# shaunlebron/blinky

Hardware: AMD Instinct MI355X
Metric: warped Mpixels/s (lensmap apply) (higher is better)
Workload: dtype u8; 1 GPU; 3840x2160 cube/panini f_fov 180, 64 frames/step from a resident ring of 64 distinct globes (1.80 GB, advanced every step), one lensmap; value / ms_per_step = the job with steps alternating between 2 HIP stream(s), value_one_stream = the same on one stream, roofline.kernel_ms_per_launch = the kernel alone under HIP events; 64 frames/step since r5 (r1-r4 ran 16: compare those with value_at_16_frames; ring_globes=64, parallelism=row-stripes x1, streams=2

## Files before the change

blinky_amd/csrc/bk_build_kernels.h:

```cpp

BK_DEV void bk_state_init(BkState &S, const BkBuildParams *P)
{
    S.P = P;
    S.err = 0;
    S.steps = 0;
    S.flag = 0;
    BK_INIT_GLOBALS(S)
}

BK_DEV int bk_ray_to_plate_index(BkState &S, const float *ray)
{
    const BkBuildParams &P = *S.P;
#ifdef BK_HAS_GLOBE_PLATE
    bkv a[3] = {bk_num((double)ray[0]), bk_num((double)ray[1]), bk_num((double)ray[2])};
    bkv r[BK_MAXRET];
    int n = LF_globe_plate(S, a, 3, r);
    if (n < 1 || !bk_isnum(r[n - 1])) return -1;
    double d = r[n - 1].n;
    if (r[n - 1].e != 0.0 && !(bkm_rint(d - r[n - 1].e) == bkm_rint(d + r[n - 1].e))) S.flag = 1;
    if (!(d > -2147483648.0 && d < 2147483647.0)) return -1;
    int plate = (int)bkm_rint(d);
    if (plate < 0 || plate >= P.numplates) return -1;
    return plate;
#else
// ... 112 lines not shown
    if (threadIdx.x < 6) s_disp[threadIdx.x] = 0;
    __syncthreads();
    const int lx = blockIdx.x * blockDim.x + threadIdx.x;
    const int lyl = blockIdx.y;
    const int ly = P.row0 + lyl;
    int err = 0;
    bool flagged = false;
    unsigned int off = 0xFFFFFFFFu;
    unsigned char tint = 255;
    unsigned short sub = 0x8080;
    const size_t o = (size_t)lyl * P.W + lx;
    if (lx < P.W) {
        int plate;
        BkState S;
        bk_state_init(S, &P);
        bk_inverse_entry(P, S, lx, ly, &off, &tint, &plate, P.subtexel ? &sub : nullptr);
        if (plate >= 0 && !S.flag) s_disp[plate] = 1;
        err = S.err;
        P.offsets[o] = off;
        P.tints[o] = tint;
        if (P.subtexel) P.subtexel[o] = sub;
        flagged = S.flag != 0;
        if ((err & BK_ERR_RESULT) && P.first_bad) atomicMax(P.first_bad, (unsigned int)(ly * P.W + (P.W - 1 - lx)) + 1u);
    }
    bk_push_flagged_wave(P, flagged, (unsigned int)o, off, tint, sub);
    __syncthreads();
    bk_publish_flags(s_disp, P.display, err, P.err);
}
#endif
#endif

// ... 404 lines not shown
```

blinky_amd/csrc/bk_emit.cpp:

```cpp
#include "bk_emit.h"

#include <cmath>
#include <cstdio>
#include <map>
#include <set>
#include <sstream>

namespace bk {
using namespace bklua;

namespace {

[[noreturn]] void unsupported(const std::string &chunk, int line, const std::string &what)
{
    throw LuaError(chunk + ":" + std::to_string(line) + ": not supported in a GPU callback: " + what);
}

std::string sanitize(const std::string &s)
{
    std::string o;
    for (char c : s) o += (isalnum((unsigned char)c) ? c : '_');
    return o;
}

// ... 14 lines not shown
};

struct Emitter {
    Interp &I;
    std::map<std::pair<const FuncProto *, std::string>, FnInfo> fns;
    std::vector<std::string> fn_code;
    std::set<std::string> mutable_globals;
    std::map<const Table *, std::pair<std::string, int>> const_tables;
    std::ostringstream table_code;
    int uid = 0;
    struct SinCos { std::string s, c; long epoch; };
    std::map<std::string, SinCos> sincos;
    long epoch = 0;
    struct Pure { std::string name; long epoch; };
    std::map<std::string, Pure> pure;
    std::string last_single, last_single_of;
    static bool is_name(const std::string &v)
    {
        if (v.empty() || (v[0] >= '0' && v[0] <= '9')) return false;
        for (char c : v) if (!(c == '_' || c == '.' || (c >= '0' && c <= '9') || (c >= 'a' && c <= 'z') || (c >= 'A' && c <= 'Z'))) return false;
        return true;
    }
    static bool mentions(const std::string &key, const std::string &var)
    {
        auto word = [](char c) { return c == '_' || c == '.' || (c >= '0' && c <= '9') || (c >= 'a' && c <= 'z') || (c >= 'A' && c <= 'Z'); };
        for (size_t at = key.find(var); at != std::string::npos; at = key.find(var, at + 1)) {
            const bool left = at == 0 || !word(key[at - 1]), right = at + var.size() >= key.size() || !word(key[at + var.size()]);
            if (left && right) return true;
        }
        return false;
// ... 16 lines not shown
    struct Scope {
        const FuncProto *proto = nullptr;
        const Closure *cl = nullptr;
        const Scope *parent = nullptr;
    };
    struct Fn : Scope {
        std::ostringstream out;
        int indent = 1;
        std::map<int, int> array_slots;
        std::map<int, std::string> fn_slots;
        std::set<int> fn_open;
        std::map<int, Value> static_slots;
        std::map<int, std::vector<std::string>> record_slots;
        std::map<int, std::pair<int, int>> matrix_slots;
        std::string lp = "l", ap = "A", rp = "R";
        std::string field_var(int slot, const std::string &name) const { return rp + std::to_string(slot) + "_" + name; }
        bool is_table(int slot) const { return array_slots.count(slot) || record_slots.count(slot) || matrix_slots.count(slot); }
        std::string chunk;
    };
    static const Value *upvalue_of(const Scope *s, int idx, const Scope **owner, int *slot)
    {
        while (!s->cl) {
            const UpvalDesc &d = s->proto->upvals[(size_t)idx];
            if (d.from_parent_local) { *owner = s->parent; *slot = d.index; return nullptr; }
            idx = d.index;
            s = s->parent;
        }
        *owner = nullptr;
        return s->cl->upvals[(size_t)idx].get();
    }
// ... 211 lines not shown
        switch (e.kind) {
        case Expr::Nil: return "bk_nil()";
        case Expr::True: return "bk_bool(true)";
        case Expr::False: return "bk_bool(false)";
        case Expr::Number: return num_literal(e.num);
        case Expr::String: return str_literal(e.str);
        case Expr::Vararg: {
            const std::string np = std::to_string(f.proto->nparams);
            return "(na > " + np + " ? a[" + np + "] : bk_nil())";
        }
        case Expr::Function: unsupported(f.chunk, e.line, "function values / closures");
        case Expr::Table: unsupported(f.chunk, e.line, "table constructors other than 'local t = {a, b, ...}'");
        case Expr::Name: {
            int slot = 0;
            if (Fn *o = local_of(f, e, &slot)) {
                if (o->is_table(slot)) unsupported(f.chunk, e.line, "table '" + e.str + "' used as a value");
                if (o->fn_slots.count(slot)) unsupported(f.chunk, e.line, "function '" + e.str + "' used as a value (a function defined inside a callback can only be called)");
                if (o->static_slots.count(slot))
                    unsupported(f.chunk, e.line, std::string(o->static_slots[slot].t == Value::TABLE ? "table" : "function") + " '" + e.str +
                                                     "' used as a value (it can be " + (o->static_slots[slot].t == Value::TABLE ? "indexed" : "called") + ", and passed on to script functions)");
                return o->lp + std::to_string(slot);
            }
            if (e.var == VarKind::Global && mutable_globals.count(e.str)) return "S.g_" + sanitize(e.str);
            if (e.var == VarKind::Upvalue) {
                const Scope *owner = nullptr;
                if (const std::string *field = cell_field(upvalue_of(&f, e.slot, &owner, &slot))) return "S." + *field;
            }
            {
                Value v;
                static_value(f, e, &v);
// ... 8 lines not shown
                const auto &names = ao->record_slots[aslot];
                for (const std::string &n : names) if (n == e.b->str) return ao->field_var(aslot, n);
                return "bk_nil()";
            }
            if (ao && ao->matrix_slots.count(aslot)) unsupported(f.chunk, e.line, "a row of table '" + e.a->str + "' used as a value");
            if (e.a->kind == Expr::Index) {
                int mslot = 0;
                Fn *mo = local_of(f, *e.a->a, &mslot);
                if (mo && mo->matrix_slots.count(mslot)) {
                    const std::string row = matrix_row(f, *mo, mslot, *e.a->b);
                    const std::string k = emit_expr(f, *e.b), t = tmp();
                    line(f, "bkv " + t + " = bk_aget(S, " + row + ", " + std::to_string(mo->matrix_slots[mslot].second) + ", " + k + ");");
                    return t;
                }
            }
            if (ao && ao->array_slots.count(aslot)) {
                std::string k = emit_expr(f, *e.b), t = tmp();
                line(f, "bkv " + t + " = bk_aget(S, " + ao->ap + std::to_string(aslot) + ", " + std::to_string(ao->array_slots[aslot]) + ", " + k + ");");
                return t;
            }
            Value sv;
            if (static_value(f, e, &sv)) return const_value(f, e, sv, "field '" + e.b->str + "'");
            Value o;
            if (static_value(f, *e.a, &o) && o.t == Value::TABLE) {
                auto ct = const_table(f, e, o.tab_ptr(), e.a->kind == Expr::Name ? e.a->str : "table");
                std::string k = emit_expr(f, *e.b), t = tmp();
                line(f, "bkv " + t + " = bk_aget(S, " + ct.first + ", " + std::to_string(ct.second) + ", " + k + ");");
                return t;
            }
            unsupported(f.chunk, e.line, "indexing this expression");
// ... 144 lines not shown
        }
        return {arr, cnt};
    }

    bool single_valued_call(Fn &f, const Expr &e)
    {
        Value callee;
        if (e.kind != Expr::Call || !e.str.empty() || !static_value(f, *e.a, &callee) || callee.t != Value::BUILTIN) return false;
        const std::string &bn = callee.bi()->name;
        return bn.compare(0, 5, "math.") == 0 && bn != "math.modf" && bn != "math.frexp";
    }

    void emit_call(Fn &f, const Expr &e, std::string *arr, std::string *cnt)
    {
        ad_call.clear();
        Value callee, self_obj;
        const bool method = !e.str.empty();
        if (method) {
            if (!static_value(f, *e.a, &self_obj) || self_obj.t != Value::TABLE)
                unsupported(f.chunk, e.line, "method calls (a:" + e.str + "(..)) on a value that is not a constant table of the script");
            callee = static_field(self_obj, Value::string(e.str));
            if (callee.t != Value::FUNC) unsupported(f.chunk, e.line, "method '" + e.str + "' is not a script function");
        } else {
            int slot = 0;
            Fn *o = local_of(f, *e.a, &slot);
            if (o && o->fn_slots.count(slot)) {
                if (o->fn_open.count(slot)) unsupported(f.chunk, e.line, "recursion ('" + e.a->str + "')");
                *arr = tmp("r");
                *cnt = tmp("n");
                Args a = emit_args(f, e.args);
                auto packed = pack(f, a, 1);
                line(f, "bkv " + *arr + "[BK_MAXRET];");
                line(f, "const int " + *cnt + " = " + o->fn_slots[slot] + "(" + packed.first + ", " + packed.second + ", " + *arr + ");");
                ++epoch;
                return;
            }
        }
        if (!method && !static_value(f, *e.a, &callee)) {
            std::string n = e.a->kind == Expr::Name ? "'" + e.a->str + "'" : "this expression";
            unsupported(f.chunk, e.line, "calling " + n + " (callee must be a script function or builtin known at build time)");
        }
        *arr = tmp("r");
        *cnt = tmp("n");
        if (callee.t == Value::FUNC) {
            std::vector<std::pair<int, Value>> bound;
            std::vector<const Expr *> plain;
            static const Expr nil_expr = [] { Expr x; x.kind = Expr::Nil; return x; }();
            const int shift = method ? 1 : 0;
            if (method) {
// ... 4 lines not shown
            for (size_t i = 0; i < e.args.size(); ++i) {
                Value av;
                const Expr &x = *e.args[i];
                if ((int)i + shift < callee.fn()->proto->nparams && (x.kind == Expr::Name || x.kind == Expr::Index) && static_value(f, x, &av) &&
                    (av.is_function() || av.t == Value::TABLE)) {
                    bound.emplace_back((int)i + shift, av);
                    plain.push_back(&nil_expr);
                } else plain.push_back(&x);
            }
            const FnInfo &fi = ensure_function(callee.fn(), e.line, f.chunk, bound);
            Args a = emit_args(f, plain);
            auto packed = pack(f, a, 1);
            line(f, "bkv " + *arr + "[BK_MAXRET];");
            line(f, "const int " + *cnt + " = " + fi.cname + "(S, " + packed.first + ", " + packed.second + ", " + *arr + ");");
            ++epoch;
            return;
        }
        if (callee.t != Value::BUILTIN) {
            std::string n = e.a->kind == Expr::Name ? e.a->str : "?";
            unsupported(f.chunk, e.line, "attempt to call '" + n + "' (a " + callee.type_name() + " value)");
        }
        const std::string &bn = callee.bi()->name;
        if (bn == "print") {
            line(f, "bkv " + *arr + "[1]; const int " + *cnt + " = 0; (void)" + *arr + ";");
            return;
        }
        Args a = emit_args(f, e.args);
        auto A = [&](size_t i) { return arg_at(a, i); };
        auto single = [&](const std::string &expr) {
            line(f, "bkv " + *arr + "[1] = {" + expr + "}; const int " + *cnt + " = 1;");
// ... 232 lines not shown
        if (ao && ao->record_slots.count(slot)) {
            if (target.b->kind != Expr::String) unsupported(f.chunk, target.line, "indexing record '" + target.a->str + "' with a computed key");
            for (const std::string &n : ao->record_slots[slot]) if (n == target.b->str) { line(f, ao->field_var(slot, n) + " = " + val + ";"); forget(ao->field_var(slot, n)); return; }
            unsupported(f.chunk, target.line, "adding field '" + target.b->str + "' to '" + target.a->str + "' (name it in the constructor)");
        }
        if (target.a->kind == Expr::Index) {
            int mslot = 0;
            Fn *mo = local_of(f, *target.a->a, &mslot);
            if (mo && mo->matrix_slots.count(mslot)) {
                const std::string row = matrix_row(f, *mo, mslot, *target.a->b);
                const std::string k = emit_expr(f, *target.b);
                line(f, "bk_aset(S, " + row + ", " + std::to_string(mo->matrix_slots[mslot].second) + ", " + k + ", " + val + ");");
                return;
            }
        }
        if (ao && ao->array_slots.count(slot)) {
            std::string k = emit_expr(f, *target.b);
            line(f, "bk_aset(S, " + ao->ap + std::to_string(slot) + ", " + std::to_string(ao->array_slots[slot]) + ", " + k + ", " + val + ");");
            return;
        }
        unsupported(f.chunk, target.line, "storing into this table (only tables created by 'local t = {..}' in the same function are writable)");
    }

    static void declare_locals(std::ostream &o, const Fn &f, const std::string &pad)
    {
        const FuncProto *p = f.proto;
        for (int i = 0; i < p->nslots; ++i) {
            if (f.fn_slots.count(i)) continue;
            if (f.record_slots.count(i)) {
                for (const std::string &name : f.record_slots.at(i)) o << pad << "bkv " << f.field_var(i, name) << " = bk_nil();   /* " << p->slot_names[i] << "." << name << " */\n";
            } else if (f.matrix_slots.count(i)) {
                const int cells = f.matrix_slots.at(i).first * f.matrix_slots.at(i).second;
                o << pad << "bkv " << f.ap << i << "[" << cells + 1 << "];   /* " << p->slot_names[i] << " */\n";
                o << pad << "for (int q = 0; q <= " << cells << "; ++q) " << f.ap << i << "[q] = bk_nil();\n";
            } else if (f.array_slots.count(i)) {
                o << pad << "bkv " << f.ap << i << "[" << f.array_slots.at(i) + 1 << "];   /* " << p->slot_names[i] << " */\n";
            } else if (i < p->nparams) {
                o << pad << "bkv " << f.lp << i << " = na > " << i << " ? a[" << i << "] : bk_nil();   /* " << p->slot_names[i] << " */\n";
            } else {
                o << pad << "bkv " << f.lp << i << " = bk_nil();   /* " << p->slot_names[i] << " */\n";
            }
        }
    }

    void emit_local_function(Fn &f, const Stmt &s)
    {
        const FuncProto *p = s.exprs[0]->proto;
        const int slot = s.slots[0];
        if (f.fn_slots.count(slot) || f.is_table(slot)) unsupported(f.chunk, s.line, "re-declaring '" + s.names[0] + "'");
        const std::string id = std::to_string(++uid);
        Fn g;
        g.proto = p;
        g.parent = &f;
        g.chunk = f.chunk;
        g.lp = "n" + id + "_l";
        g.ap = "n" + id + "_A";
        g.rp = "n" + id + "_R";
        g.indent = f.indent + 1;
        const std::string name = "NF" + id + "_" + sanitize(s.names[0]);
        f.fn_slots[slot] = name;
        f.fn_open.insert(slot);
        emit_block(g, p->body);
        f.fn_open.erase(slot);
        line(f, "/* " + f.chunk + ":" + std::to_string(p->line) + "  function " + s.names[0] + " */");
        line(f, "auto " + name + " = [&](const bkv *a, int na, bkv *r) -> int {");
        std::ostringstream decl;
        declare_locals(decl, g, std::string((size_t)(f.indent + 1) * 4, ' '));
        f.out << decl.str();
        line(f, "    (void)a; (void)na; (void)r;");
        f.out << g.out.str();
        line(f, "    return 0;");
        line(f, "};");
    }

    void emit_stmt(Fn &f, const Stmt &s)
    {
        const bool plain = s.kind == Stmt::Local || s.kind == Stmt::Assign;
        if (!plain) ++epoch;
        emit_stmt_body(f, s);
        if (!plain) ++epoch;
    }
    void emit_stmt_body(Fn &f, const Stmt &s)
    {
        switch (s.kind) {
        case Stmt::Local: {
            if (s.slots.size() == 1 && s.exprs.size() == 1 && s.exprs[0]->kind == Expr::Function) { emit_local_function(f, s); return; }
            if (s.slots.size() == 1 && s.exprs.size() == 1 && (s.exprs[0]->kind == Expr::Name || s.exprs[0]->kind == Expr::Index)) {
// ... 41 lines not shown
                return;
            }
            if (s.slots.size() == 1 && s.exprs.size() == 1 && s.exprs[0]->kind == Expr::Table) {
                const Expr &t = *s.exprs[0];
                if (!t.fields.empty()) unsupported(f.chunk, s.line, "table constructors mixing positional and named fields");
                if (!t.args.empty() && t.args.back()->kind == Expr::Call && !single_valued_call(f, *t.args.back()))
                    unsupported(f.chunk, s.line, "call expansion inside a table constructor (write '(f(...))' to keep one value)");
                if (!t.args.empty() && t.args.back()->kind == Expr::Vararg)
                    unsupported(f.chunk, s.line, "'...' at the end of a table constructor (a table of a size only known at run time)");
                std::vector<std::string> vals;
                for (auto &x : t.args) vals.push_back(emit_expr(f, *x));
                int n = (int)vals.size();
                if (f.array_slots.count(s.slots[0]) && f.array_slots[s.slots[0]] != n) unsupported(f.chunk, s.line, "re-declaring a table with a different size");
                if (f.record_slots.count(s.slots[0]) || f.matrix_slots.count(s.slots[0])) unsupported(f.chunk, s.line, "re-declaring a table");
                f.array_slots[s.slots[0]] = n;
                for (int i = 0; i < n; ++i) line(f, f.ap + std::to_string(s.slots[0]) + "[" + std::to_string(i + 1) + "] = " + vals[i] + ";");
                return;
            }
            auto v = emit_values(f, s.exprs, s.slots.size());
            for (size_t i = 0; i < s.slots.size(); ++i) {
                line(f, f.lp + std::to_string(s.slots[i]) + " = " + v[i] + ";");
                forget(f.lp + std::to_string(s.slots[i]));
                if (ad_active && &f == ad_fn && ad_slot.count(s.slots[i])) line(f, ad_slot[s.slots[i]] + " = " + d_of(v[i]) + ";");
            }
            return;
        }
        case Stmt::LocalFunction: emit_local_function(f, s); return;
        case Stmt::Assign: {
            auto v = emit_values(f, s.exprs, s.targets.size());
            for (size_t i = 0; i < s.targets.size(); ++i) store(f, *s.targets[i], v[i]);
            return;
// ... 3 lines not shown
            line(f, "{");
            f.indent++;
            emit_call(f, *s.call, &arr, &cnt);
            line(f, "(void)" + cnt + ";");
            f.indent--;
            line(f, "}");
            return;
        }
        case Stmt::Do:
            line(f, "{");
            f.indent++;
            emit_block(f, s.body);
            f.indent--;
            line(f, "}");
            return;
        case Stmt::While: {
            line(f, "for (;;) {");
            f.indent++;
            line(f, "if (!bk_tick(S)) break;");
            std::string c = emit_expr(f, *s.cond);
            line(f, "if (!bk_truthy(" + c + ")) break;");
            emit_block(f, s.body);
            f.indent--;
            line(f, "}");
            return;
        }
        case Stmt::Repeat: {
            line(f, "for (;;) {");
            f.indent++;
            line(f, "if (!bk_tick(S)) break;");
            emit_block(f, s.body);
            std::string c = emit_expr(f, *s.cond);
            line(f, "if (bk_truthy(" + c + ")) break;");
            f.indent--;
            line(f, "}");
            return;
        }
        case Stmt::If: {
            int opened = 0;
            for (size_t i = 0; i < s.clauses.size(); ++i) {
                const auto &c = s.clauses[i];
                if (!c.first) {
                    emit_block(f, c.second);
                    break;
                }
                std::string cv = emit_expr(f, *c.first);
                line(f, "if (bk_truthy(" + cv + ")) {");
                f.indent++;
                emit_block(f, c.second);
                f.indent--;
// ... 78 lines not shown
            line(f, "const bkv " + gv + " = " + arr + "[" + gi + "];");
            line(f, std::string("if (") + gv + ".t == BK_TNIL) " + (is_ipairs ? "break;" : "continue;"));
            for (size_t i = 0; i < s.slots.size(); ++i)
                line(f, f.lp + std::to_string(s.slots[i]) + " = " + (i == 0 ? "bk_num((double)" + gi + ")" : i == 1 ? gv : std::string("bk_nil()")) + ";");
            emit_block(f, s.body);
            f.indent--;
            line(f, "}");
            return;
        }
        case Stmt::Return: {
            if (s.exprs.size() == 1 && s.exprs[0]->kind == Expr::Call) {
                std::string arr, cnt;
                line(f, "{");
                f.indent++;
                emit_call(f, *s.exprs[0], &arr, &cnt);
                line(f, "for (int q = 0; q < " + cnt + "; ++q) r[q] = " + arr + "[q];");
                line(f, "return " + cnt + ";");
                f.indent--;
                line(f, "}");
                return;
            }
            line(f, "{");
            f.indent++;
            Args a = emit_args(f, s.exprs);
            if (a.fixed.size() > 8) unsupported(f.chunk, s.line, "more than 8 return values");
            if (a.multi && a.fixed.size() > 4) unsupported(f.chunk, s.line, "more than 4 return values in front of a trailing call or `...`");
            for (size_t i = 0; i < a.fixed.size(); ++i) line(f, "r[" + std::to_string(i) + "] = " + a.fixed[i] + ";");
            if (a.multi) {
                line(f, "for (int q = 0; q < " + a.mcnt + " && " + std::to_string(a.fixed.size()) + " + q < BK_MAXRET; ++q) r[" + std::to_string(a.fixed.size()) + " + q] = " + a.marr + "[q];");
                line(f, "return " + std::to_string(a.fixed.size()) + " + " + a.mcnt + ";");
            } else line(f, "return " + std::to_string(a.fixed.size()) + ";");
// ... 22 lines not shown
        if (fi.emitting) unsupported(from_chunk, line_no, "recursion ('" + cl->proto->name + "')");
        fi.proto = cl->proto;
        fi.cl = cl;
        fi.cname = "LF" + std::to_string(++uid) + "_" + sanitize(cl->proto->name);
        fi.emitting = true;

        Fn f;
        f.proto = cl->proto;
        f.cl = cl;
        f.chunk = cl->chunk->name;
        for (auto &b : bound) {
            if (!slot_is_constant(cl->proto, b.first))
                unsupported(from_chunk, line_no, std::string(b.second.t == Value::TABLE ? "a table" : "a function") + " passed as '" + cl->proto->slot_names[(size_t)b.first] + "' of '" + cl->proto->name + "', which assigns or captures that parameter");
            f.static_slots[b.first] = b.second;
        }
        emit_block(f, cl->proto->body);

        std::ostringstream o;
        o << "/* " << f.chunk << ":" << cl->proto->line << "  function " << cl->proto->name << " */\n";
        o << "BK_DEV int " << fi.cname << "(BkState &S, const bkv *a, int na, bkv *r)\n{\n";
        declare_locals(o, f, "    ");
        o << "    (void)a; (void)na; (void)r;\n";
        o << f.out.str();
        o << "    return 0;\n}\n\n";
        fn_code.push_back(o.str());
        fi.emitting = false;
        fi.done = true;
        return fi;
    }
};
// ... 355 lines not shown
```

blinky_amd/csrc/bk_lens.cpp:

```cpp
#include <chrono>
#include <cstring>
#include <future>

#include "bk_emit.h"
#include "bk_lens_priv.h"

using namespace bklua;

namespace bk {

static double need_num(const Values &a, size_t i, const char *fn)
{
    if (i >= a.size() || a[i].t != Value::NUM)
        throw LuaError(std::string("bad argument #") + std::to_string(i + 1) + " to '" + fn + "' (number expected)");
    return a[i].n;
}

LensProgram::LensProgram(bk_ctx *ctx) : interp(math_platform())
{
    interp.print_sink = [this](const std::string &s) { console += s; };
    static const char *alias[] = {"cos", "sin", "tan", "asin", "acos", "atan", "atan2", "sinh", "cosh", "tanh",
                                  "log", "log10", "abs", "sqrt", "exp", "pow"};
    Value math = interp.get_global("math");
    for (const char *a : alias) interp.set_global(a, math.tab()->get(Value::string(a)));
// ... 395 lines not shown
extern "C" int bk_debug_kernel_source(bk_ctx *ctx, char *buf, size_t cap, size_t *needed, int compile)
{
    if (!ctx) return BK_E_INVALID;
    LensProgram *P = ctx->prog;
    if (!P || !P->lens_valid) return ctx->fail(BK_E_STATE, "no valid lens");
    std::string src;
    if (int r = generate_source(ctx, P, &src)) return r;
    if (needed) *needed = src.size() + 1;
    if (buf && cap) snprintf(buf, cap, "%s", src.c_str());
    if (compile) return compile_module(ctx, P, src);
    return BK_OK;
}
#endif

#if BK_DEBUG_API
extern "C" int bk_debug_eval(bk_ctx *ctx, int which, const double *args, int nargs, double *out, int *nout)
{
    if (!ctx || !ctx->prog) return BK_E_INVALID;
    LensProgram *P = ctx->prog;
    const Value &f = which == 0 ? P->lens_inverse : which == 1 ? P->lens_forward : P->globe_plate;
    if (!f.is_function()) return ctx->fail(BK_E_STATE, "callback not defined");
    try {
        Values a;
        for (int i = 0; i < nargs; ++i) a.push_back(Value::number(args[i]));
        P->interp.steps = 0;
        Values r = P->interp.call(f, a);
        *nout = (int)r.size();
        for (size_t i = 0; i < r.size() && i < 8; ++i) out[i] = r[i].t == Value::NUM ? r[i].n : __builtin_nan("");
        if (r.size() == 1 && r[0].t == Value::NIL) *nout = -1;
    } catch (const LuaError &e) {
// ... 27 lines not shown
```

blinky_amd/csrc/bk_modules.cpp:

```cpp
#include <hip/hiprtc.h>

#include <cerrno>
#include <chrono>
#include <cstring>
#include <map>
#include <mutex>
#include <dlfcn.h>
#include <fcntl.h>
#include <spawn.h>
#include <sys/stat.h>
#include <sys/wait.h>
#include <unistd.h>

#include "bk_codecache.h"
#include "bk_emit.h"
#include "bk_modules.h"

using namespace bk;
extern char **environ;

static std::string cache_path(const std::string &source, const std::string &arch)
{
    const std::string dir = cache_dir();
    if (dir.empty()) return std::string();
    Sha256 h;
    h.update(source);
    for (int i = 0; i < bk::kNumEmbeddedHeaders; ++i) h.update(std::string(bk::kEmbeddedHeaders[i].text));
    h.update(arch);
    h.update(std::string(bk_version()));
    h.update(std::string("-O3 -std=c++17 -ffp-contract=off"));
    return dir + "/bk_lens_" + hex128(h) + ".hsaco";
}

static std::mutex g_rtc_mutex;
static std::map<uint64_t, std::shared_ptr<std::vector<char>>> g_rtc_cache;

static uint64_t code_key(const std::string &source, const std::string &arch)
{
    return fnv1a64(arch.data(), arch.size(), fnv1a64(source.data(), source.size()));
}

CodeResult cached_code(const std::string &source, const std::string &arch)
{
    CodeResult r;
    std::lock_guard<std::mutex> lock(g_rtc_mutex);
// ... 15 lines not shown
    CodeResult r = cached_code(source, arch);
    if (r.code) return r;
    std::lock_guard<std::mutex> lock(g_rtc_mutex);
    auto hit = g_rtc_cache.find(code_key(source, arch));
    if (hit != g_rtc_cache.end() && !bk::g_debug.no_memcache) { r.code = hit->second; return r; }
    std::vector<const char *> hnames, htexts;
    for (int i = 0; i < bk::kNumEmbeddedHeaders; ++i) {
        hnames.push_back(bk::kEmbeddedHeaders[i].name);
        htexts.push_back(bk::kEmbeddedHeaders[i].text);
    }
    hiprtcProgram prog;
    if (hiprtcCreateProgram(&prog, source.c_str(), "bk_lens_build.hip", (int)hnames.size(), htexts.data(), hnames.data()) != HIPRTC_SUCCESS) {
        r.rc = BK_E_HIP; r.log = "hiprtcCreateProgram failed";
        return r;
    }
    const char *opts[] = {arch.c_str(), "-O3", "-std=c++17", "-ffp-contract=off"};
    if (hiprtcCompileProgram(prog, 4, opts) != HIPRTC_SUCCESS) {
        size_t n = 0;
        hiprtcGetProgramLogSize(prog, &n);
        std::string log(n, 0);
        if (n) hiprtcGetProgramLog(prog, &log[0]);
        hiprtcDestroyProgram(&prog);
        r.rc = BK_E_HIP; r.log = "hiprtc failed to compile the lens kernels: " + log;
        return r;
    }
    size_t cs = 0;
    hiprtcGetCodeSize(prog, &cs);
    r.code = std::make_shared<std::vector<char>>(cs);
    hiprtcGetCode(prog, r.code->data());
    hiprtcDestroyProgram(&prog);
    store_sealed(cache_path(source, arch), *r.code);
    if (g_rtc_cache.size() >= 64) g_rtc_cache.clear();
// ... 179 lines not shown
```

blinky_amd/ffi.py:

```python
import ctypes as C
import os

import numpy as np

try:
    import torch
except ImportError:
    torch = None

LIB_PATH = os.environ.get("BLINKY_HIP_LIB") or os.path.join(os.path.dirname(os.path.abspath(__file__)), "libblinkyhip.so")
if not os.path.exists(LIB_PATH):
    raise ImportError(
        f"{LIB_PATH} is missing: build it with `python -c 'import __graft_entry__ as g; g.build()'` "
        "(or `make -C blinky_amd/csrc`).  There is no CPU fallback."
    )
lib = C.CDLL(LIB_PATH)

MAX_PLATES = 6
MIP_MAX_LEVELS = 16
NULL_OFFSET = 0xFFFFFFFF
DEVICE_NONE = -2
OK = 0
PENDING = 1
MAP_NONE, MAP_INVERSE, MAP_FORWARD = 0, 1, 2
# ... 83 lines not shown
    "bk_create_palmap": (None, [_vp, _vp]),
    "bk_create_tintmap_rgba": (None, [_vp, _vp]),
    "bk_get_size": (_i, [_vp] + [C.POINTER(_i)] * 5),
    "bk_version": (C.c_char_p, []),
    "bk_set_apply_variant": (_i, [_vp, _i]),
    "bk_set_resident_share": (_i, [_vp, _i, _i, _i]),
    "bk_set_resident_apply": (_i, [_vp, _i]),
    "bk_multi_set_resident_apply": (_i, [_vp, _i]),
    "bk_set_blockmap_tuning": (_i, [_vp, _i]),
    "bk_set_host_compile": (_i, [_i]),
    "bk_host_module_ready": (_i, [_vp, _i]),
    "bk_debug_module_from_cache": (_i, [_vp]),
    "bk_debug_forward_tiles": (_i, [_vp, C.POINTER(_i), C.POINTER(_i)]),
    "bk_debug_set_option": (_i, [C.c_char_p, _i]),
    "bk_debug_build_breakdown": (_i, [_vp, C.POINTER(_d)]),
    "bk_multi_lensmap_valid": (_i, [_vp]),
    "bk_last_build_ms": (_d, [_vp]),
    "bk_globe_pitch": (_i, [_vp]),
    "bk_globe_rows": (_i, [_vp]),
    "bk_globe_texel_offset": (C.c_uint32, [_vp, _i, _i, _i]),
    "bk_download_plate": (_i, [_vp, _i, _i, _vp, _i]),
    "bk_save_plate": (_i, [_vp, _i, _i, _i, _vp, _i]),
    "bk_debug_tile_stats": (_i, [_vp, C.POINTER(_i)]),
    "bk_debug_traffic_model": (_i, [_vp, C.POINTER(C.c_uint64)]),
    "bk_debug_band_balance": (_i, [_vp, C.POINTER(C.c_uint32)]),
    "bk_debug_stream_mix": (_i, [_vp, _sz, _i, _i, C.POINTER(_d)]),
    "bk_debug_fnv1a64": (_i, [_vp, _sz, C.POINTER(C.c_uint64)]),
    "bk_debug_host_build": (_i, [_vp, _i, _vp, _vp, C.POINTER(_i), C.POINTER(_d)]),
    "bk_debug_host_build_subtexel": (_i, [_vp, _i, _vp, _vp, _vp, C.POINTER(_i), C.POINTER(_d)]),
    "bk_debug_resident_latency": (_i, [_vp, _i, _vp, _i, _i, C.POINTER(_d), C.POINTER(_d)]),
# ... 41 lines not shown
    "bk_multi_clear_globe": (_i, [_vp]),
    "bk_multi_resize": (_i, [_vp, _i, _i]),
    "bk_multi_set_frames": (_i, [_vp, _i]),
    "bk_multi_set_zoom": (_i, [_vp, _i, _i]),
    "bk_multi_set_rubixgrid": (_i, [_vp, _i, _d, _d]),
    "bk_multi_upload_plate": (_i, [_vp, _i, _i, _vp, _i]),
    "bk_multi_fill_plate_lcg": (_i, [_vp, _i, _i, C.c_uint32]),
    "bk_multi_synchronize": (_i, [_vp]),
    "bk_multi_build": (_i, [_vp, C.POINTER(_i), C.POINTER(_d)]),
    "bk_multi_apply": (_i, [_vp, _i, _vp, _i, _i, _i, _i, _vp]),
    "bk_multi_apply_stripes": (_i, [_vp, _i, _i, C.POINTER(_vp), _i, _vp]),
    "bk_multi_wait": (_i, [_vp, _i]),
    "bk_multi_gather": (_i, [_vp, C.POINTER(_vp), _i, _i, _vp, _sz, _i]),
    "bk_multi_exchange_rotating": (_i, [_vp, C.POINTER(_vp), _i, C.POINTER(_vp), _sz, _i]),
}
for _name, (_res, _args) in _SIGS.items():
    _fn = getattr(lib, _name)
    _fn.restype, _fn.argtypes = _res, _args

EXPORTS = tuple(_SIGS)


class BlinkyError(RuntimeError):
    pass


def debug_set_option(name, value):
    if lib.bk_debug_set_option(name.encode(), int(value)) != OK:
        raise ValueError(f"bk_debug_set_option: unknown option {name!r}")


# ... 115 lines not shown
    def calc_zoom(self):
        scale = _d()
        self._chk(lib.bk_calc_zoom(self._h, C.byref(scale)))
        return scale.value

    def last_build_fixups(self):
        a, b = _i(), _i()
        self._chk(lib.bk_last_build_fixups(self._h, C.byref(a), C.byref(b)))
        return a.value, b.value

    def build_breakdown(self):
        out = (_d * 6)()
        self._chk(lib.bk_debug_build_breakdown(self._h, out))
        return dict(build_ms=out[0], host_eval_ms=out[1], flagged=int(out[2]), pool_threads=int(out[3]), kernel_wall_ms=out[4],
                    retries=int(out[5]) % 1000, compiled_host_module=out[5] >= 1000)

    def host_build(self, mode=0):
        W, H, ps, r0, r1 = self.size()
        off = np.empty((r1 - r0) * W, np.uint32)
        tin = np.empty((r1 - r0) * W, np.uint8)
        disp = (_i * MAX_PLATES)()
        scale = _d()
        rc = lib.bk_debug_host_build(self._h, int(mode), _ptr(off), _ptr(tin), disp, C.byref(scale))
        err = None
        if rc != OK:
            err = lib.bk_last_error(self._h).decode(errors="replace")
            if rc != -3:
                raise BlinkyError(f"[{rc}] {err}")
        return off, tin, list(disp), scale.value, err

# ... 610 lines not shown
```

include/blinky_hip_debug.h:

```cpp
#ifndef BLINKY_HIP_DEBUG_H
#define BLINKY_HIP_DEBUG_H

#include "blinky_hip.h"

#ifdef __cplusplus
extern "C" {
#endif

int         bk_debug_set_option(const char *name, int value);
int         bk_debug_module_from_cache(const bk_ctx *ctx);
int         bk_debug_forward_tiles(bk_ctx *ctx, int *taken, int *total);
int         bk_debug_set_ablation(bk_ctx *ctx, int bits);
int         bk_debug_tile_stats(bk_ctx *ctx, int out[6]);
int         bk_debug_traffic_model(bk_ctx *ctx, uint64_t out[8]);
int         bk_debug_band_balance(bk_ctx *ctx, uint32_t out[18]);
int         bk_debug_stream_mix(bk_ctx *ctx, size_t bytes, int period, int writes, double *gbps);
int         bk_debug_host_build(bk_ctx *ctx, int mode, uint32_t *offsets, uint8_t *tints, int display_out[BK_MAX_PLATES], double *scale_out);
int         bk_debug_host_build_subtexel(bk_ctx *ctx, int mode, uint32_t *offsets, uint8_t *tints, uint16_t *sub, int display_out[BK_MAX_PLATES],
                                         double *scale_out);
int         bk_debug_fnv1a64(const void *host, size_t bytes, uint64_t *out);
int         bk_debug_resident_latency(bk_ctx *ctx, int frames, void *dst_dev, int dst_pitch, int globes, double *host_us, double *device_us);
int         bk_debug_xcd_of_workgroups(bk_ctx *ctx, int *out, int nworkgroups);
int         bk_debug_set_tile_shape(bk_ctx *ctx, int lw);
int         bk_debug_kernel_source(bk_ctx *ctx, char *buf, size_t cap, size_t *needed, int compile);
int         bk_debug_build_params(bk_ctx *ctx, void *out, size_t cap, size_t *needed);
int         bk_debug_host_entries(bk_ctx *ctx, const uint32_t *ids, size_t n, uint32_t *offsets, uint8_t *tints);
int         bk_debug_host_corners(bk_ctx *ctx, const uint32_t *ids, size_t n, int32_t *sx, int32_t *sy, uint8_t *ok);
int         bk_debug_set_forward_corners(bk_ctx *ctx, const int32_t *xy, const uint8_t *ok, size_t ncorners);
int         bk_debug_eval(bk_ctx *ctx, int which, const double *args, int nargs, double out[8], int *nout);
int         bk_debug_eval_device(bk_ctx *ctx, int which, const double *args, int nargs, int n, double *out, int *nout);
int         bk_debug_eval_device_bounds(bk_ctx *ctx, int which, const double *args, int nargs, int n, double *out, double *bound, int *flag,
                                        int *nout);
int         bk_debug_build_breakdown(const bk_ctx *ctx, double out[6]);
int         bk_debug_stripe_bounds(const uint32_t *row_cost, int H, int W, int nranks, int *bounds_out);
int         bk_debug_row_costs(bk_ctx *ctx, uint32_t *host_out);
long long   bk_debug_fb_decode_check(int gp, int ph);
int         bk_debug_mip_pyramid(bk_ctx *ctx, const void *const plates_dev[BK_MAX_PLATES], const int plate_pitch_bytes[BK_MAX_PLATES]);

#ifdef __cplusplus
}
#endif
#endif
```

Baseline: 2.722 million Mpixels/s.

## Unroll counted Lua loops and scalarize small tables in generated lens build kernels

The Lua-to-HIP emitter now detects while/repeat loops with a literal-initialized counter and a constant bound, fully unrolls them, and replaces small local tables indexed only by that counter with individual scalar variables instead of indexed arrays. The build kernel always passes a local subtexel slot, and the RTC compile adds a flag that disables common-code sinking in simplifycfg. The aim is to avoid dynamic indexing into private arrays that spill to scratch and to lower register and control-flow cost in the lensmap build kernel. This targets the build path, not the per-frame apply kernel that the metric measures, so throughput is likely unchanged. Unrolling raises code size and a debug query for kernel register and scratch usage is added.

```diff
diff --git a/blinky_amd/csrc/bk_build_kernels.h b/blinky_amd/csrc/bk_build_kernels.h
--- a/blinky_amd/csrc/bk_build_kernels.h
+++ b/blinky_amd/csrc/bk_build_kernels.h
@@ -150,7 +150,9 @@
         int plate;
         BkState S;
         bk_state_init(S, &P);
-        bk_inverse_entry(P, S, lx, ly, &off, &tint, &plate, P.subtexel ? &sub : nullptr);
+        unsigned short entry_sub = 0x8080;
+        bk_inverse_entry(P, S, lx, ly, &off, &tint, &plate, &entry_sub);
+        if (P.subtexel) sub = entry_sub;
         if (plate >= 0 && !S.flag) s_disp[plate] = 1;
         err = S.err;
         P.offsets[o] = off;
diff --git a/blinky_amd/csrc/bk_emit.cpp b/blinky_amd/csrc/bk_emit.cpp
--- a/blinky_amd/csrc/bk_emit.cpp
+++ b/blinky_amd/csrc/bk_emit.cpp
@@ -52,6 +52,7 @@
     long epoch = 0;
     struct Pure { std::string name; long epoch; };
     std::map<std::string, Pure> pure;
+    bool call_of_script = false;
     std::string last_single, last_single_of;
     static bool is_name(const std::string &v)
     {
@@ -98,6 +99,15 @@
         std::map<int, std::vector<std::string>> record_slots;
         std::map<int, std::pair<int, int>> matrix_slots;
         std::string lp = "l", ap = "A", rp = "R";
+        struct Unrolled {
+            int counter = -1;
+            std::vector<int> heads;
+            std::set<int> stops;
+        };
+        std::map<const Stmt *, Unrolled> unrolled;
+        std::set<int> scalar_slots;
+        std::map<int, int> counter_now;
+        std::string element_var(int slot, int k) const { return ap + std::to_string(slot) + "_" + std::to_string(k); }
         std::string field_var(int slot, const std::string &name) const { return rp + std::to_string(slot) + "_" + name; }
         bool is_table(int slot) const { return array_slots.count(slot) || record_slots.count(slot) || matrix_slots.count(slot); }
         std::string chunk;
@@ -339,6 +349,7 @@
         case Expr::Name: {
             int slot = 0;
             if (Fn *o = local_of(f, e, &slot)) {
+                if (o == &f && f.counter_now.count(slot)) return num_literal((double)f.counter_now[slot]);
                 if (o->is_table(slot)) unsupported(f.chunk, e.line, "table '" + e.str + "' used as a value");
                 if (o->fn_slots.count(slot)) unsupported(f.chunk, e.line, "function '" + e.str + "' used as a value (a function defined inside a callback can only be called)");
                 if (o->static_slots.count(slot))
@@ -377,6 +388,7 @@
                     return t;
                 }
             }
+            if (ao && ao->scalar_slots.count(aslot)) return element_get(f, *ao, aslot, *e.b);
             if (ao && ao->array_slots.count(aslot)) {
                 std::string k = emit_expr(f, *e.b), t = tmp();
                 line(f, "bkv " + t + " = bk_aget(S, " + ao->ap + std::to_string(aslot) + ", " + std::to_string(ao->array_slots[aslot]) + ", " + k + ");");
@@ -551,6 +563,7 @@
     void emit_call(Fn &f, const Expr &e, std::string *arr, std::string *cnt)
     {
         ad_call.clear();
+        call_of_script = false;
         Value callee, self_obj;
         const bool method = !e.str.empty();
         if (method) {
@@ -570,6 +583,7 @@
                 line(f, "bkv " + *arr + "[BK_MAXRET];");
                 line(f, "const int " + *cnt + " = " + o->fn_slots[slot] + "(" + packed.first + ", " + packed.second + ", " + *arr + ");");
                 ++epoch;
+                call_of_script = true;
                 return;
             }
         }
@@ -604,6 +618,7 @@
             line(f, "bkv " + *arr + "[BK_MAXRET];");
             line(f, "const int " + *cnt + " = " + fi.cname + "(S, " + packed.first + ", " + packed.second + ", " + *arr + ");");
             ++epoch;
+            call_of_script = true;
             return;
         }
         if (callee.t != Value::BUILTIN) {
@@ -866,6 +881,7 @@
                 return;
             }
         }
+        if (ao && ao->scalar_slots.count(slot)) { element_set(f, *ao, slot, *target.b, val); return; }
         if (ao && ao->array_slots.count(slot)) {
             std::string k = emit_expr(f, *target.b);
             line(f, "bk_aset(S, " + ao->ap + std::to_string(slot) + ", " + std::to_string(ao->array_slots[slot]) + ", " + k + ", " + val + ");");
@@ -885,6 +901,10 @@
                 const int cells = f.matrix_slots.at(i).first * f.matrix_slots.at(i).second;
                 o << pad << "bkv " << f.ap << i << "[" << cells + 1 << "];   /* " << p->slot_names[i] << " */\n";
                 o << pad << "for (int q = 0; q <= " << cells << "; ++q) " << f.ap << i << "[q] = bk_nil();\n";
+            } else if (f.scalar_slots.count(i) && f.array_slots.count(i)) {
+                o << pad << "bkv ";
+                for (int k = 1; k <= f.array_slots.at(i); ++k) o << (k > 1 ? ", " : "") << f.element_var(i, k);
+                o << ";   /* " << p->slot_names[i] << " */\n";
             } else if (f.array_slots.count(i)) {
                 o << pad << "bkv " << f.ap << i << "[" << f.array_slots.at(i) + 1 << "];   /* " << p->slot_names[i] << " */\n";
             } else if (i < p->nparams) {
@@ -912,6 +932,7 @@
         const std::string name = "NF" + id + "_" + sanitize(s.names[0]);
         f.fn_slots[slot] = name;
         f.fn_open.insert(slot);
+        plan_unroll(g);
         emit_block(g, p->body);
         f.fn_open.erase(slot);
         line(f, "/* " + f.chunk + ":" + std::to_string(p->line) + "  function " + s.names[0] + " */");
@@ -923,6 +944,346 @@
         f.out << g.out.str();
         line(f, "    return 0;");
         line(f, "};");
+    }
+
+    static constexpr int kUnrollCap = 256;
+
+    static const Expr &unparen(const Expr &e)
+    {
+        const Expr *x = &e;
+        while (x->kind == Expr::Unop && x->str == "()") x = x->a.get();
+        return *x;
+    }
+    static bool int_literal(const Expr &e0, int *v)
+    {
+        const Expr &e = unparen(e0);
+        if (e.kind == Expr::Unop && e.str == "-") {
+            if (!int_literal(*e.a, v) || *v == 0) return false;
+            *v = -*v;
+            return true;
+        }
+        if (e.kind != Expr::Number || e.num != std::floor(e.num) || std::fabs(e.num) > 1e6) return false;
+        *v = (int)e.num;
+        return true;
+    }
+    static bool counter_step(const Stmt &s, int *slot, int *step)
+    {
+        if (s.kind != Stmt::Assign || s.targets.size() != 1 || s.exprs.size() != 1) return false;
+        const Expr &t = *s.targets[0], &x = unparen(*s.exprs[0]);
+        if (t.kind != Expr::Name || t.var != VarKind::Local || x.kind != Expr::Binop || (x.str != "+" && x.str != "-")) return false;
+        const Expr &a = unparen(*x.a);
+        int k = 0;
+        if (a.kind != Expr::Name || a.var != VarKind::Local || a.slot != t.slot || !int_literal(*x.b, &k) || k == 0) return false;
+        *slot = t.slot;
+        *step = x.str == "+" ? k : -k;
+        return true;
+    }
+    static bool index_of(const Expr &e0, int *counter, int *off)
+    {
+        const Expr &e = unparen(e0);
+        if (int_literal(e, off)) { *counter = -1; return true; }
+        if (e.kind == Expr::Name && e.var == VarKind::Local) { *counter = e.slot; *off = 0; return true; }
+        if (e.kind == Expr::Binop && (e.str == "+" || e.str == "-")) {
+            const Expr &a = unparen(*e.a);
+            int k = 0;
+            if (a.kind == Expr::Name && a.var == VarKind::Local && int_literal(*e.b, &k)) { *counter = a.slot; *off = e.str == "+" ? k : -k; return true; }
+        }
+        return false;
+    }
+    struct Bound { char op = 0; int K = 0; };
+    static bool holds(const Bound &b, int v) { return b.op == '<' ? v < b.K : b.op == 'l' ? v <= b.K : b.op == '>' ? v > b.K : b.op == 'g' ? v >= b.K : v == b.K; }
+    static bool bound_of(const Expr &e0, int slot, Bound *b)
+    {
+        const Expr &e = unparen(e0);
+        if (e.kind != Expr::Binop) return false;
+        const char op = e.str == "<" ? '<' : e.str == "<=" ? 'l' : e.str == ">" ? '>' : e.str == ">=" ? 'g' : e.str == "==" ? '=' : 0;
+        const Expr &a = unparen(*e.a);
+        if (!op || a.kind != Expr::Name || a.var != VarKind::Local || a.slot != slot || !int_literal(*e.b, &b->K)) return false;
+        b->op = op;
+        return true;
+    }
+    static void chain(const Expr &e0, const char *op, std::vector<const Expr *> *out)
+    {
+        const Expr &e = unparen(e0);
+        if (e.kind == Expr::Binop && e.str == op) { chain(*e.a, op, out); chain(*e.b, op, out); }
+        else out->push_back(&e);
+    }
+    static int count_stmts(const Block &b)
+    {
+        int n = 0;
+        for (const StmtP &s : b) {
+            n += 1 + count_stmts(s->body);
+            for (auto &c : s->clauses) n += count_stmts(c.second);
+        }
+        return n;
+    }
+
+    struct UnrollScan {
+        std::set<int> not_counter;
+        std::map<int, int> tables;
+        std::set<int> not_scalar;
+        struct Use { int table, counter; const Stmt *top; };
+        std::vector<Use> uses;
+    };
+    static void scan_assignments(UnrollScan &u, const Block &b, int where)
+    {
+        for (const StmtP &sp : b) {
+            const Stmt &s = *sp;
+            int v = 0, slot = 0, step = 0;
+            if (s.kind == Stmt::Local) {
+                if (!(where == 0 && s.slots.size() == 1 && s.exprs.size() == 1 && int_literal(*s.exprs[0], &v)))
+                    for (int sl : s.slots) u.not_counter.insert(sl);
+                if (s.slots.size() == 1 && s.exprs.size() == 1 && s.exprs[0]->kind == Expr::Table) {
+                    const Expr &t = *s.exprs[0];
+                    if (where == 0 && t.fields.empty() && !t.args.empty() && t.args[0]->kind != Expr::Table) u.tables[s.slots[0]] = (int)t.args.size();
+                }
+            } else if (s.kind == Stmt::Assign) {
+                const bool init = where == 0 && s.targets.size() == 1 && s.exprs.size() == 1 && int_literal(*s.exprs[0], &v);
+                if (!init && !(where == 1 && counter_step(s, &slot, &step)))
+                    for (auto &t : s.targets) if (t->kind == Expr::Name && t->var == VarKind::Local) u.not_counter.insert(t->slot);
+            } else for (int sl : s.slots) u.not_counter.insert(sl);
+            scan_assignments(u, s.body, where == 0 && (s.kind == Stmt::While || s.kind == Stmt::Repeat) ? 1 : 2);
+            for (auto &c : s.clauses) scan_assignments(u, c.second, 2);
+        }
+    }
+    static void scan_uses(UnrollScan &u, const Expr *e, const Stmt *top)
+    {
+        if (!e) return;
+        if (e->kind == Expr::Index && e->a->kind == Expr::Name && e->a->var == VarKind::Local && u.tables.count(e->a->slot)) {
+            int c = 0, off = 0;
+            if (!index_of(*e->b, &c, &off)) u.not_scalar.insert(e->a->slot);
+            else if (c >= 0) u.uses.push_back({e->a->slot, c, top});
+            scan_uses(u, e->b.get(), top);
+            return;
+        }
+        if (e->kind == Expr::Name && e->var == VarKind::Local && u.tables.count(e->slot)) u.not_scalar.insert(e->slot);
+        if (e->kind == Expr::Function) return;
+        scan_uses(u, e->a.get(), top);
+        scan_uses(u, e->b.get(), top);
+        for (auto &x : e->args) scan_uses(u, x.get(), top);
+        for (auto &x : e->fields) { scan_uses(u, x.first.get(), top); scan_uses(u, x.second.get(), top); }
+    }
+    static void scan_uses(UnrollScan &u, const Block &b, const Stmt *top)
+    {
+        for (const StmtP &sp : b) {
+            const Stmt &s = *sp;
+            const Stmt *t = top ? top : &s;
+            for (auto &x : s.targets) scan_uses(u, x.get(), t);
+            for (auto &x : s.exprs) scan_uses(u, x.get(), t);
+            scan_uses(u, s.call.get(), t);
+            scan_uses(u, s.cond.get(), t);
+            scan_uses(u, s.body, t);
+            for (auto &c : s.clauses) { scan_uses(u, c.first.get(), t); scan_uses(u, c.second, t); }
+        }
+    }
+    static bool plan_loop(const Stmt &s, int slot, int step, const std::set<int> &entries, Fn::Unrolled *plan, std::set<int> *after, bool *open)
+    {
+        std::vector<const Expr *> parts;
+        chain(*s.cond, s.kind == Stmt::While ? "and" : "or", &parts);
+        Bound b;
+        bool found = false;
+        for (const Expr *x : parts) {
+            Bound c;
+            if (found || !bound_of(*x, slot, &c)) continue;
+            const bool up = c.op == '>' || c.op == 'g', down = c.op == '<' || c.op == 'l';
+            if (s.kind == Stmt::While ? (down && step > 0) || (up && step < 0) : c.op == '=' || (up && step > 0) || (down && step < 0)) { b = c; found = true; }
+        }
+        if (!found) return false;
+        std::set<int> heads;
+        for (int e : entries) {
+            if (s.kind == Stmt::Repeat && b.op == '=' && !((b.K - e) % step == 0 && (b.K - e) / step >= 1)) { *open = true; continue; }
+            int v = e;
+            for (int n = 0;; ++n, v += step) {
+                if (n > kUnrollCap) return false;
+                heads.insert(v);
+                after->insert(v);
+                if (s.kind == Stmt::While) {
+                    if (!holds(b, v)) { plan->stops.insert(v); break; }
+                } else {
+                    after->insert(v + step);
+                    if (holds(b, v + step)) break;
+                }
+            }
+        }
+        if (heads.empty()) return false;
+        plan->counter = slot;
+        plan->heads.assign(heads.begin(), heads.end());
+        if (step < 0) plan->heads.assign(heads.rbegin(), heads.rend());
+        return true;
+    }
+    void plan_unroll(Fn &f)
+    {
+        const FuncProto *p = f.proto;
+        UnrollScan u;
+        scan_assignments(u, p->body, 0);
+        if (u.tables.empty()) return;
+        scan_uses(u, p->body, nullptr);
+        auto counter_ok = [&](int slot) { return slot >= p->nparams && !p->is_captured(slot) && !u.not_counter.count(slot); };
+        for (auto &t : u.tables) if (p->is_captured(t.first)) u.not_scalar.insert(t.first);
+        std::map<int, std::set<int>> vals;
+        std::map<const Stmt *, Fn::Unrolled> plans;
+        for (const StmtP &sp : p->body) {
+            const Stmt &s = *sp;
+            int v = 0;
+            if (s.kind == Stmt::Local && s.slots.size() == 1 && s.exprs.size() == 1 && int_literal(*s.exprs[0], &v)) vals[s.slots[0]] = {v};
+            else if (s.kind == Stmt::Assign && s.targets.size() == 1 && s.exprs.size() == 1 && s.targets[0]->kind == Expr::Name &&
+                     s.targets[0]->var == VarKind::Local && int_literal(*s.exprs[0], &v)) vals[s.targets[0]->slot] = {v};
+            else if (s.kind == Stmt::While || s.kind == Stmt::Repeat) {
+                std::map<int, int> steps, times;
+                for (const StmtP &bs : s.body) {
+                    int slot = 0, step = 0;
+                    if (counter_step(*bs, &slot, &step)) { steps[slot] += step; times[slot]++; }
+                }
+                int counter = -1;
+                for (auto &st : steps) {
+                    const int slot = st.first;
+                    Fn::Unrolled plan;
+                    std::set<int> after;
+                    bool open = false;
+                    if (counter < 0 && times[slot] == 1 && counter_ok(slot) && vals.count(slot) && plan_loop(s, slot, st.second, vals[slot], &plan, &after, &open) &&
+                        (int)plan.heads.size() * (1 + count_stmts(s.body)) <= kUnrollCap) {
+                        counter = slot;
+                        plans[&s] = plan;
+                        if (open) vals.erase(slot); else vals[slot] = after;
+                    } else {
+                        u.not_counter.insert(slot);
+                        vals.erase(slot);
+                    }
+                }
+            }
+        }
+        for (bool changed = true; changed;) {
+            changed = false;
+            for (auto it = plans.begin(); it != plans.end();) {
+                bool keep = counter_ok(it->second.counter), any = false;
+                for (const auto &use : u.uses)
+                    if (use.top == it->first && use.counter == it->second.counter) { any = true; keep = keep && !u.not_scalar.count(use.table); }
+                if (keep && any) { ++it; continue; }
+                u.not_counter.insert(it->second.counter);
+                it = plans.erase(it);
+                changed = true;
+            }
+            for (const auto &use : u.uses) {
+                if (u.not_scalar.count(use.table)) continue;
+                bool ok = counter_ok(use.counter);
+                const Stmt::Kind k = use.top->kind;
+                if (ok && (k == Stmt::While || k == Stmt::Repeat || k == Stmt::NumFor || k == Stmt::GenFor)) {
+                    auto pl = plans.find(use.top);
+                    ok = pl != plans.end() && pl->second.counter == use.counter;
+                }
+                if (!ok) { u.not_scalar.insert(use.table); changed = true; }
+            }
+        }
+        for (const auto &use : u.uses)
+            if (plans.count(use.top) && !u.not_scalar.count(use.table)) f.scalar_slots.insert(use.table);
+        f.unrolled = plans;
+    }
+
+    bool static_index(Fn &f, const Expr &e, int *k)
+    {
+        int c = 0, off = 0;
+        if (!index_of(e, &c, &off)) return false;
+        if (c < 0) { *k = off; return true; }
+        auto now = f.counter_now.find(c);
+        if (now == f.counter_now.end()) return false;
+        *k = now->second + off;
+        return true;
+    }
+    std::string element_get(Fn &f, Fn &o, int slot, const Expr &index)
+    {
+        const int n = o.array_slots[slot];
+        int k = 0;
+        if (static_index(f, index, &k)) {
+            const std::string t = tmp();
+            line(f, "bkv " + t + " = " + (k >= 1 && k <= n ? o.element_var(slot, k) : std::string("bk_nil()")) + ";");
+            return t;
+        }
+        const std::string kx = emit_expr(f, index), ki = tmp("k"), t = tmp();
+        line(f, "const bkv " + ki + " = " + kx + "; bk_need_exact(S, " + ki + ");");
+        line(f, "bkv " + t + " = bk_nil();");
+        std::string sel;
+        for (k = 1; k <= n; ++k) sel += std::string(k > 1 ? "else " : "") + "if (" + ki + ".n == " + std::to_string(k) + ".0) " + t + " = " + o.element_var(slot, k) + "; ";
+        line(f, "if (" + ki + ".t == BK_TNUM) { " + sel + "}");
+        return t;
+    }
+    void element_set(Fn &f, Fn &o, int slot, const Expr &index, const std::string &val)
+    {
+        const int n = o.array_slots[slot];
+        int k = 0;
+        if (static_index(f, index, &k)) {
+            if (k >= 1 && k <= n) { line(f, o.element_var(slot, k) + " = " + val + ";"); forget(o.element_var(slot, k)); }
+            else line(f, "S.err |= BK_ERR_INDEX;");
+            return;
+        }
+        const std::string kx = emit_expr(f, index), ki = tmp("k");
+        line(f, "const bkv " + ki + " = " + kx + "; bk_need_exact(S, " + ki + ");");
+        std::string sel;
+        for (k = 1; k <= n; ++k) {
+            sel += "if (" + ki + ".t == BK_TNUM && " + ki + ".n == " + std::to_string(k) + ".0) " + o.element_var(slot, k) + " = " + val + "; else ";
+            forget(o.element_var(slot, k));
+        }
+        line(f, sel + "S.err |= BK_ERR_INDEX;");
+    }
+
+    void emit_loop(Fn &f, const Stmt &s)
+    {
+        line(f, "for (;;) {");
+        f.indent++;
+        line(f, "if (!bk_tick(S)) break;");
+        if (s.kind == Stmt::While) {
+            std::string c = emit_expr(f, *s.cond);
+            line(f, "if (!bk_truthy(" + c + ")) break;");
+            emit_block(f, s.body);
+        } else {
+            emit_block(f, s.body);
+            std::string c = emit_expr(f, *s.cond);
+            line(f, "if (bk_truthy(" + c + ")) break;");
+        }
+        f.indent--;
+        line(f, "}");
+    }
+    void emit_copy(Fn &f, const Block &body, int counter)
+    {
+        ++epoch;
+        for (const StmtP &sp : body) {
+            int slot = 0, step = 0;
+            if (counter_step(*sp, &slot, &step) && slot == counter) {
+                const std::string L = f.lp + std::to_string(counter);
+                f.counter_now[counter] += step;
+                line(f, L + " = " + num_literal((double)f.counter_now[counter]) + ";");
+                forget(L);
+            } else emit_stmt(f, *sp);
+        }
+        ++epoch;
+    }
+    void emit_unrolled(Fn &f, const Stmt &s, const Fn::Unrolled &u)
+    {
+        const std::string L = f.lp + std::to_string(u.counter);
+        line(f, "do {     /* " + f.chunk + ":" + std::to_string(s.line) + "  one copy of the loop's trip per value of " + f.proto->slot_names[(size_t)u.counter] + ", then the loop */");
+        f.indent++;
+        for (int v : u.heads) {
+            line(f, "if (" + L + ".t == BK_TNUM && " + L + ".e == 0.0 && " + L + ".n == " + std::to_string(v) + ".0) {");
+            f.indent++;
+            f.counter_now[u.counter] = v;
+            line(f, "if (!bk_tick(S)) break;");
+            if (s.kind == Stmt::While) {
+                ++epoch;
+                const std::string c = emit_expr(f, *s.cond);
+                line(f, "if (!bk_truthy(" + c + ")) break;");
+                if (!u.stops.count(v)) emit_copy(f, s.body, u.counter);
+            } else {
+                emit_copy(f, s.body, u.counter);
+                const std::string c = emit_expr(f, *s.cond);
+                line(f, "if (bk_truthy(" + c + ")) break;");
+            }
+            f.counter_now.erase(u.counter);
+            ++epoch;
+            f.indent--;
+            line(f, "}");
+        }
+        emit_loop(f, s);
+        f.indent--;
+        line(f, "} while (0);");
     }
 
     void emit_stmt(Fn &f, const Stmt &s)
@@ -994,7 +1355,9 @@
                 if (f.array_slots.count(s.slots[0]) && f.array_slots[s.slots[0]] != n) unsupported(f.chunk, s.line, "re-declaring a table with a different size");
                 if (f.record_slots.count(s.slots[0]) || f.matrix_slots.count(s.slots[0])) unsupported(f.chunk, s.line, "re-declaring a table");
                 f.array_slots[s.slots[0]] = n;
-                for (int i = 0; i < n; ++i) line(f, f.ap + std::to_string(s.slots[0]) + "[" + std::to_string(i + 1) + "] = " + vals[i] + ";");
+                const bool scalars = f.scalar_slots.count(s.slots[0]) != 0;
+                for (int i = 0; i < n; ++i)
+                    line(f, (scalars ? f.element_var(s.slots[0], i + 1) : f.ap + std::to_string(s.slots[0]) + "[" + std::to_string(i + 1) + "]") + " = " + vals[i] + ";");
                 return;
             }
             auto v = emit_values(f, s.exprs, s.slots.size());
@@ -1028,26 +1391,11 @@
             f.indent--;
             line(f, "}");
             return;
-        case Stmt::While: {
-            line(f, "for (;;) {");
-            f.indent++;
-            line(f, "if (!bk_tick(S)) break;");
-            std::string c = emit_expr(f, *s.cond);
-            line(f, "if (!bk_truthy(" + c + ")) break;");
-            emit_block(f, s.body);
-            f.indent--;
-            line(f, "}");
-            return;
-        }
+        case Stmt::While:
         case Stmt::Repeat: {
-            line(f, "for (;;) {");
-            f.indent++;
-            line(f, "if (!bk_tick(S)) break;");
-            emit_block(f, s.body);
-            std::string c = emit_expr(f, *s.cond);
-            line(f, "if (bk_truthy(" + c + ")) break;");
-            f.indent--;
-            line(f, "}");
+            auto plan = f.unrolled.find(&s);
+            if (plan != f.unrolled.end()) emit_unrolled(f, s, plan->second);
+            else emit_loop(f, s);
             return;
         }
         case Stmt::If: {
@@ -1156,7 +1504,8 @@
                 line(f, "{");
                 f.indent++;
                 emit_call(f, *s.exprs[0], &arr, &cnt);
-                line(f, "for (int q = 0; q < " + cnt + "; ++q) r[q] = " + arr + "[q];");
+                if (call_of_script) line(f, "for (int q = 0; q < BK_MAXRET; ++q) if (q < " + cnt + ") r[q] = " + arr + "[q];");
+                else line(f, "for (int q = 0; q < " + cnt + "; ++q) r[q] = " + arr + "[q];");
                 line(f, "return " + cnt + ";");
                 f.indent--;
                 line(f, "}");
@@ -1209,6 +1558,7 @@
                 unsupported(from_chunk, line_no, std::string(b.second.t == Value::TABLE ? "a table" : "a function") + " passed as '" + cl->proto->slot_names[(size_t)b.first] + "' of '" + cl->proto->name + "', which assigns or captures that parameter");
             f.static_slots[b.first] = b.second;
         }
+        plan_unroll(f);
         emit_block(f, cl->proto->body);
 
         std::ostringstream o;
diff --git a/blinky_amd/csrc/bk_lens.cpp b/blinky_amd/csrc/bk_lens.cpp
--- a/blinky_amd/csrc/bk_lens.cpp
+++ b/blinky_amd/csrc/bk_lens.cpp
@@ -433,6 +433,22 @@
 #endif
 
 #if BK_DEBUG_API
+extern "C" int bk_debug_build_kernel_info(bk_ctx *ctx, int out[4])
+{
+    if (!ctx || !out) return BK_E_INVALID;
+    LensProgram *P = ctx->prog;
+    if (!P || !P->module) return ctx->fail(BK_E_STATE, "no lens module is loaded (bk_build first)");
+    hipFunction_t fn = P->k_inverse ? P->k_inverse : P->k_corners;
+    if (!fn) return ctx->fail(BK_E_STATE, "the lens module has no build kernel");
+    BK_HIP(ctx, hipFuncGetAttribute(&out[0], HIP_FUNC_ATTRIBUTE_NUM_REGS, fn));
+    BK_HIP(ctx, hipFuncGetAttribute(&out[1], HIP_FUNC_ATTRIBUTE_LOCAL_SIZE_BYTES, fn));
+    BK_HIP(ctx, hipFuncGetAttribute(&out[2], HIP_FUNC_ATTRIBUTE_SHARED_SIZE_BYTES, fn));
+    out[3] = P->k_inverse ? 1 : 2;
+    return BK_OK;
+}
+#endif
+
+#if BK_DEBUG_API
 extern "C" int bk_debug_eval(bk_ctx *ctx, int which, const double *args, int nargs, double *out, int *nout)
 {
     if (!ctx || !ctx->prog) return BK_E_INVALID;
diff --git a/blinky_amd/csrc/bk_modules.cpp b/blinky_amd/csrc/bk_modules.cpp
--- a/blinky_amd/csrc/bk_modules.cpp
+++ b/blinky_amd/csrc/bk_modules.cpp
@@ -19,6 +19,8 @@
 using namespace bk;
 extern char **environ;
 
+static const char kRtcOptionsText[] = "-O3 -std=c++17 -ffp-contract=off -mllvm -simplifycfg-sink-common=false";
+
 static std::string cache_path(const std::string &source, const std::string &arch)
 {
     const std::string dir = cache_dir();
@@ -28,7 +30,7 @@
     for (int i = 0; i < bk::kNumEmbeddedHeaders; ++i) h.update(std::string(bk::kEmbeddedHeaders[i].text));
     h.update(arch);
     h.update(std::string(bk_version()));
-    h.update(std::string("-O3 -std=c++17 -ffp-contract=off"));
+    h.update(std::string(kRtcOptionsText));
     return dir + "/bk_lens_" + hex128(h) + ".hsaco";
 }
 
@@ -74,8 +76,8 @@
         r.rc = BK_E_HIP; r.log = "hiprtcCreateProgram failed";
         return r;
     }
-    const char *opts[] = {arch.c_str(), "-O3", "-std=c++17", "-ffp-contract=off"};
-    if (hiprtcCompileProgram(prog, 4, opts) != HIPRTC_SUCCESS) {
+    const char *opts[] = {arch.c_str(), "-O3", "-std=c++17", "-ffp-contract=off", "-mllvm", "-simplifycfg-sink-common=false"};
+    if (hiprtcCompileProgram(prog, 6, opts) != HIPRTC_SUCCESS) {
         size_t n = 0;
         hiprtcGetProgramLogSize(prog, &n);
         std::string log(n, 0);
diff --git a/blinky_amd/ffi.py b/blinky_amd/ffi.py
--- a/blinky_amd/ffi.py
+++ b/blinky_amd/ffi.py
@@ -121,6 +121,7 @@
     "bk_debug_forward_tiles": (_i, [_vp, C.POINTER(_i), C.POINTER(_i)]),
     "bk_debug_set_option": (_i, [C.c_char_p, _i]),
     "bk_debug_build_breakdown": (_i, [_vp, C.POINTER(_d)]),
+    "bk_debug_build_kernel_info": (_i, [_vp, C.POINTER(_i)]),
     "bk_multi_lensmap_valid": (_i, [_vp]),
     "bk_last_build_ms": (_d, [_vp]),
     "bk_globe_pitch": (_i, [_vp]),
@@ -192,7 +193,10 @@
     "bk_multi_gather": (_i, [_vp, C.POINTER(_vp), _i, _i, _vp, _sz, _i]),
     "bk_multi_exchange_rotating": (_i, [_vp, C.POINTER(_vp), _i, C.POINTER(_vp), _sz, _i]),
 }
+_AB_MAY_LACK = {"bk_debug_build_kernel_info"}
 for _name, (_res, _args) in _SIGS.items():
+    if _name in _AB_MAY_LACK and os.environ.get("BLINKY_HIP_LIB") and not hasattr(lib, _name):
+        continue
     _fn = getattr(lib, _name)
     _fn.restype, _fn.argtypes = _res, _args
 
@@ -338,6 +342,13 @@
         self._chk(lib.bk_debug_build_breakdown(self._h, out))
         return dict(build_ms=out[0], host_eval_ms=out[1], flagged=int(out[2]), pool_threads=int(out[3]), kernel_wall_ms=out[4],
                     retries=int(out[5]) % 1000, compiled_host_module=out[5] >= 1000)
+
+    def build_kernel_info(self):
+        if not hasattr(lib, "bk_debug_build_kernel_info"):
+            return None
+        out = (_i * 4)()
+        self._chk(lib.bk_debug_build_kernel_info(self._h, out))
+        return dict(vgprs=out[0], scratch_bytes=out[1], lds_bytes=out[2], kind=out[3])
 
     def host_build(self, mode=0):
         W, H, ps, r0, r1 = self.size()
diff --git a/include/blinky_hip_debug.h b/include/blinky_hip_debug.h
--- a/include/blinky_hip_debug.h
+++ b/include/blinky_hip_debug.h
@@ -32,6 +32,7 @@
 int         bk_debug_eval_device_bounds(bk_ctx *ctx, int which, const double *args, int nargs, int n, double *out, double *bound, int *flag,
                                         int *nout);
 int         bk_debug_build_breakdown(const bk_ctx *ctx, double out[6]);
+int         bk_debug_build_kernel_info(bk_ctx *ctx, int out[4]);
 int         bk_debug_stripe_bounds(const uint32_t *row_cost, int H, int W, int nranks, int *bounds_out);
 int         bk_debug_row_costs(bk_ctx *ctx, uint32_t *host_out);
 long long   bk_debug_fb_decode_check(int gp, int ph);
```

After: 2.721 million Mpixels/s, median of 3. Within noise of the previous version (-0.0%).
